# vacp2p/zerokit

Hardware: AMD Instinct MI355X
Metric: RLN Groth16 proofs/sec (BN254, h=20) (higher is better)
Workload: dtype u32 limbs (256-bit Montgomery integers, BN254 Fr/Fq; 8x32 and 9x29 forms)

## Files before the change

### zerokit_amd/csrc/prover.hip

```cpp
#include "prover.h"

#include <fcntl.h>
#include <stdlib.h>
#include <string.h>
#include <sys/stat.h>
#include <time.h>
#include <unistd.h>

#include <algorithm>
#include <atomic>
#include <chrono>
#include <deque>
#include <mutex>
#include <thread>

#include "prover_kernels.h"
#include "prover_plan.h"
#include "fq29.h"
#include "glv.h"
#include "pairing.h"
#include "poseidon.h"
#include "witness_ops.h"
#include "witness_lanes.h"
#include "witness_sched.h"
// ... 126 lines not shown
  hipStream_t sA = nullptr, sAb = nullptr, sA2 = nullptr, sB = nullptr, sB2 = nullptr, sC = nullptr;
  hipStream_t sV = nullptr;
  hipStream_t sW = nullptr;
  uint32_t seq = 0;
  hipStream_t st[ST_COUNT] = {};
  StreamPlan splan;
  float ms[PROVER_STAGES] = {0};
  DevBuf<unsigned long long> walk_clk;
  ProverTuning tune;
  DeviceCount device;
  DevBuf<GNode29> nodes29;
  DevBuf<uint32_t> consts29, slot2node;
  WitLanes witlanes;
  uint32_t nstore29 = 0, nprog29 = 0;

  uint32_t N = 0, NS = 0, NI = 0, nc = 0, ni = 0, n = 0;
  int logn = 0;
  DevBuf<uint32_t> sig2node;
  DevBuf<uint32_t> a_ptr, a_col, b_ptr, b_col;
  DevBuf<uint32_t> mv_long;
  uint32_t n_mv_long = 0;
  DevBuf<Fr> a_coef, b_coef;
  DevBuf<Fr> tw_f, tw_i, coset;
  DevBuf<G1Affine29> t1_29;
  DevBuf<G2Affine29> t2_29;
  DevBuf<uint32_t> sid1, sid2;
  struct Plan {
    DevBuf<uint32_t> rows, rsid, early_ids, late_ids, prows, prsid, pout;
    DevBuf<ChunkDesc> chunks, groups, segs, segchunks, segblocks, pchunks;
    uint32_t nchunks = 0, ngroups = 0, nseg = 0, n_early = 0, n_late = 0, npchunks = 0, nblocks = 0, maxblk = 0;
    void upload(const WalkPlan& W, hipStream_t s) {
      nchunks = (uint32_t)W.chunks.size();
      ngroups = (uint32_t)W.groups.size();
      nseg = W.nseg;
      n_early = (uint32_t)W.early_ids.size();
      n_late = (uint32_t)W.late_ids.size();
      npchunks = (uint32_t)W.pchunks.size();
      nblocks = W.nblocks;
      maxblk = W.maxblk;
      rows.assign(W.rows, s);
      rsid.assign(W.rsid, s);
      chunks.assign(W.chunks, s);
      groups.assign(W.groups, s);
      segs.assign(W.segs, s);
      segchunks.assign(W.segchunks, s);
      segblocks.assign(W.segblocks, s);
// ... 172 lines not shown
  t.verify_lanes = env_int("RLNAMD_VERIFY_LANES", 0);
  if (t.verify_lanes != 1 && t.verify_lanes != 8) t.verify_lanes = 0;
  {
    const unsigned hw = std::thread::hardware_concurrency();
    const int dflt = hw ? (int)std::min<unsigned>(t.hint_threads, std::max(1u, hw / 2)) : (int)t.hint_threads;
    t.hint_threads = (uint32_t)std::min(std::max(1, env_int("RLNAMD_HINT_THREADS", dflt)), 64);
  }
  t.hint_max_warm = (uint32_t)std::min<int>(std::max(0, env_int("RLNAMD_HINTS_WARM", (int)t.hint_max_warm)), (int)HINT_PROOFS);
  t.hint_chains = (uint32_t)std::min(std::max(0, env_int("RLNAMD_HINT_CHAINS", (int)t.hint_chains)), 1024);
  return t;
}
std::string ProverTuning::describe() const {
  char b[768];
  snprintf(b, sizeof b,
           "window_bits=%d slots=%d lanechunk=%u lanechunk_walk=%u witlanes_max=%u tiny=%u ntt_lg_max=%u partial_cache=%u lone=%d "
           "lone_small=%u hints=%u hints_warm=%u hint_threads=%u hint_chains=%u verify_lanes=%d stream_shape=%s hw_queues=%d",
           window_bits, slots, lanechunk_max, lanechunk_walk_max, witlanes_max, tiny_max, ntt_lg_max, partial_cache, lone,
           lone_small_max, hint_max, hint_max_warm, hint_threads, hint_chains, verify_lanes, stream_shape_name(stream_shape), hw_queues);
  return b;
}
const ProverTuning& Prover::tuning() const { return d_->tune; }
int Prover::device_shared() const { return (d_->device.dev >= 0 && g_provers_on_device[d_->device.dev] > 1 ? 1 : 0) | (d_->device.other_process() ? 2 : 0); }

static uint32_t bitrev(uint32_t x, int bits) {
  uint32_t r = 0;
  for (int i = 0; i < bits; i++) r |= ((x >> i) & 1u) << (bits - 1 - i);
  return r;
}

static thread_local float g_init_ms[4];
static float ms_since(std::chrono::steady_clock::time_point t0) {
  return std::chrono::duration<float, std::milli>(std::chrono::steady_clock::now() - t0).count();
}
template <class F, class Entry>
static void build_table29(const std::vector<Affine<F>>& pts, const WinSched& ws, DevBuf<Entry>& table, hipStream_t s,
                          uint32_t npaired = 0) {
  size_t npts = pts.size();
  const size_t stride = ws.stride;
  auto t_alloc = std::chrono::steady_clock::now();
  table.alloc(npts * stride);
  g_init_ms[1] += ms_since(t_alloc);
  auto t_build = std::chrono::steady_clock::now();
  DevBuf<Affine<F>> d_pts(npts);
  d_pts.upload(pts.data(), npts, s);
  size_t per_pt = stride / 2 * sizeof(F);
  size_t slab = std::max<size_t>(2, (((size_t)4 << 30) / per_pt) & ~(size_t)1);
  slab = std::min(slab, (npts + 1) & ~(size_t)1);
  DevBuf<F> scratch(slab * stride / 2);
  DevBuf<Affine<F>> tmp(slab * stride);
  for (size_t k0 = 0; k0 < npts; k0 += slab) {
    size_t cnt = std::min(slab, npts - k0);
    const size_t nrows = cnt * ws.W;
// ... 126 lines not shown
      for (size_t k = 0; k < m[r].col.size(); k++) {
        hc.push_back(graph_.signals[m[r].col[k]]);
        hv.push_back(m[r].coeff[k]);
      }
      hp[r + 1] = (uint32_t)hc.size();
    }
    ptr.assign(hp, s);
    col.assign(hc, s);
    coef.assign(hv, s);
    RLN_HIP(hipStreamSynchronize(s));
  };
  csr(zk_.a, D.a_ptr, D.a_col, D.a_coef);
  csr(zk_.b, D.b_ptr, D.b_col, D.b_coef);
  {
    std::vector<uint32_t> lr;
    for (uint32_t r = 0; r < D.nc; r++)
      if (zk_.a[r].col.size() > MV_LONG || zk_.b[r].col.size() > MV_LONG) lr.push_back(r);
    D.n_mv_long = (uint32_t)lr.size();
    D.mv_long.assign(lr, s);
    RLN_HIP(hipStreamSynchronize(s));
  }

  {
    Fr root28 = Fr::from_canonical(FR_ROOT_2_28);
    Fr g = root28;
    for (int i = 0; i < 28 - (D.logn + 1); i++) g = g.sqr();
    Fr w = g.sqr();
    Fr wi = w.inv();
    std::vector<Fr> tf(D.n / 2), ti(D.n / 2), cs(D.n);
    Fr a = Fr::one(), b = Fr::one();
    for (uint32_t k = 0; k < D.n / 2; k++) {
      tf[k] = a;
      ti[k] = b;
      a = a * w;
      b = b * wi;
    }
    Fr ninv = Fr::from_u32(D.n).inv();
    std::vector<Fr> gp(D.n);
    Fr acc = ninv;
    for (uint32_t i = 0; i < D.n; i++) {
      gp[i] = acc;
      acc = acc * g;
    }
    for (uint32_t pos = 0; pos < D.n; pos++) cs[pos] = gp[bitrev(pos, D.logn)];
    D.tw_f.assign(tf, s);
    D.tw_i.assign(ti, s);
    D.coset.assign(cs, s);
    RLN_HIP(hipStreamSynchronize(s));
  }

  {
    std::vector<uint8_t> node_known = wl_known_nodes(graph_);
    D.known.resize(D.NS);
    for (uint32_t i = 0; i < D.NS; i++) D.known[i] = node_known[graph_.signals[i]];
    {
      std::vector<uint32_t> io(96);
      for (uint32_t i = 0; i < 96; i++) io[i] = i;
      D.iota96.assign(io, s);
      RLN_HIP(hipStreamSynchronize(s));
    }
    const long want = cfg.partial_cache >= 0 ? cfg.partial_cache : (long)D.tune.partial_cache;
    D.tune.partial_cache = (uint32_t)std::max(0l, want);
    if (D.witlanes.ok && want > 0) {
      const WlCone C = wl_cone(graph_, std::move(node_known));
      std::vector<uint32_t> rows;
      for (uint32_t i = 0; i < W29.slot2node.size(); i++)
        if (C.node_known[W29.slot2node[i]]) rows.push_back(i);
      D.cone.build(C.graph, wl_cone_store_slots(C, W29.store_slot), D.nstore29, s);
      D.cone_nodes = (uint32_t)C.node_of.size();
      if (D.cone.ok && !rows.empty()) {
// ... 169 lines not shown
size_t Prover::g1_rows() const { return d_->npts1; }
size_t Prover::g2_rows() const { return d_->npts2; }

void Prover::upload(size_t n, const uint8_t* inputs, const uint8_t* rs) {
  if (n > B_) throw Error("batch larger than the prover workspace (max_batch)");
  Impl& D = *d_;
  D.sync_all();
  RLN_HIP(hipMemcpyAsync(D.inputs.p, inputs, n * D.NI * 32, hipMemcpyHostToDevice, D.sA));
  RLN_HIP(hipMemcpyAsync(D.rs.p, rs, n * 64, hipMemcpyHostToDevice, D.sA));
  RLN_HIP(hipStreamSynchronize(D.sA));
}

void Prover::upload_witness(size_t n, const uint8_t* w_le) {
  if (n > B_) throw Error("batch larger than the prover workspace (max_batch)");
  Impl& D = *d_;
  D.sync_all();
  size_t words = n * (size_t)D.NS * 8;
  if (D.wgiven.n < words) D.wgiven.alloc(words);
  RLN_HIP(hipMemcpyAsync(D.wgiven.p, w_le, words * 4, hipMemcpyHostToDevice, D.sA));
  RLN_HIP(hipStreamSynchronize(D.sA));
  D.wgiven_n = n;
}

template <bool DIF>
static void launch_ntt(Fr* data, const Fr* tw, int logn, const Fr* final_scale, uint32_t B, uint32_t nb, hipStream_t s) {
  int s0 = 0;
  while (s0 < logn) {
    const int rem = logn - s0;
    const int K = rem > 3 ? 3 : rem;
    const uint32_t groups = (1u << logn) >> K;
    dim3 block(64, 1), grid(div_up(nb, 64), groups, 3);
    const Fr* sc = (s0 + K == logn) ? final_scale : nullptr;
    switch (K) {
      case 1: hipLaunchKernelGGL((k_ntt_pass<1, DIF>), grid, block, 0, s, data, tw, logn, s0, sc, B, nb); break;
      case 2: hipLaunchKernelGGL((k_ntt_pass<2, DIF>), grid, block, 0, s, data, tw, logn, s0, sc, B, nb); break;
      default: hipLaunchKernelGGL((k_ntt_pass<3, DIF>), grid, block, 0, s, data, tw, logn, s0, sc, B, nb); break;
    }
    RLN_HIP(hipGetLastError());
    s0 += K;
  }
}

void Prover::run_async(size_t n, int mode) { enqueue(n, mode, nullptr, nullptr, nullptr); }

uint64_t Prover::submit(size_t n, const uint8_t* inputs, const uint8_t* rs, int mode, const uint8_t* partial320) {
  if (n == 0) throw Error("empty batch");
  if (!inputs || !rs) throw Error("submit: inputs and rs are required");
  if (mode == PROVE_FINISH && !partial320) throw Error("submit: finish mode needs the partial points");
  return enqueue(n, mode, inputs, rs, partial320);
}

uint64_t Prover::submit_finish(size_t n, const uint8_t* inputs, const uint8_t* rs, const uint8_t* partial320,
                               const uint64_t* handles) {
  if (n == 0) throw Error("empty batch");
  if (!inputs || !rs || !partial320) throw Error("submit_finish: inputs, rs and the partial points are required");
  return enqueue(n, PROVE_FINISH, inputs, rs, partial320, handles);
}

uint32_t Prover::hint_words() const {
  const Impl& D = *d_;
  return D.segs.ok && D.tune.hint_max > 0 ? D.n_hints * 8 : 0;
}
// ... 441 lines not shown
  } else {
    hipLaunchKernelGGL(k_witness29<false>, dim3(pg), dim3(64), WIT29_LDS_BYTES, sA, D.nodes29.p, D.nprog29,
                       D.consts29.p, (uint32_t)graph_.constants.size(), in_p, D.NI, S.V29.p, S.err.p, B, nbp, nullptr);
  }
  if (small)
    hipLaunchKernelGGL(k_v29_to_fr, dim3(div_up(D.nstore29, 64), nb), dim3(64, 1), 0, sA, S.V29.p, D.slot2node.p,
                       D.nstore29, S.V.p, B, nb, 1u);
  else
    hipLaunchKernelGGL(k_v29_to_fr, dim3(pg, D.nstore29), dim3(64, 1), 0, sA, S.V29.p, D.slot2node.p, D.nstore29, S.V.p,
                       B, nbp);
  if (hinted)
    hipLaunchKernelGGL(k_hint_check, dim3(div_up(D.n_cut, 64), nb), dim3(64), 0, sA, S.V.p, D.cut_node.p, D.cut_hint.p, D.n_cut,
                       S.h_hints, D.n_hints, B, S.err.p);
  if (D.wgiven_n) {
    if (D.wgiven_n != n || mode != PROVE_FULL) throw Error("upload_witness: the next run must be a full proof of the same batch");
    hipLaunchKernelGGL(k_scatter_witness, dim3(pg, div_up(D.NS, 4)), dim3(64, 4), 0, sA, D.wgiven.p, D.sig2node.p,
                       D.NS, S.V.p, S.err.p, B, nb);
    D.wgiven_n = 0;
  }
  RLN_HIP(hipEventRecord(S.evX, sA));
  if (early) {
    hipStream_t sR1 = sA, sR3 = lone ? D.sB : sA;
    hipLaunchKernelGGL(k_recode, dim3(div_up(D.NS + 3, 64), nb), dim3(64, 1), 0, sR1, S.V.p, D.sig2node.p, D.NS,
                       S.abc.p, D.n, rs_p, D.ws, D.ws2, S.digits.p, S.digits2.p, B, nb, 1u, 1u, dB);
    if (lone) {
      RLN_HIP(hipEventRecord(S.evW, sA));
      RLN_HIP(hipStreamWaitEvent(D.sB, S.evW, 0));
    }
    if (fused)
      hipLaunchKernelGGL(k_recode, dim3(div_up(2 * D.NS + 1, 64), nb), dim3(64, 1), 0, sR3, S.V.p, D.sig2node.p, D.NS,
                         S.abc.p, D.n, rs_p, D.ws, D.ws2, S.digits.p, S.digits2.p, B, nb, 3u, 1u, dB);
    if (!lone) {
      RLN_HIP(hipEventRecord(S.evW, sA));
      RLN_HIP(hipStreamWaitEvent(D.sB, S.evW, 0));
      RLN_HIP(hipStreamWaitEvent(D.sB2, S.evW, 0));
    }
    MARK(14, D.sB);
    walk1(D.sB, P1.early_ids.p, P1.n_early);
    RLN_HIP(hipEventRecord(S.evE, D.sB));
  }
  MARK(2, sA);
  const bool values_front = sh.values_front;
  if (values_front) {
    MARK(0, sA);
    hipLaunchKernelGGL(k_values_from_witness, dim3(pg, 5), dim3(64), 0, sA, S.V.p, D.sig2node.p, B, nbp, S.values.p);
    MARK(13, sA);
    RLN_HIP(hipEventRecord(S.evV, sA));
  }
  if (sA2 != sA) RLN_HIP(hipStreamWaitEvent(sA2, S.evX, 0));
  MARK(12, sA2);
  if (mode != PROVE_PARTIAL) {
    CsrView A{D.a_ptr.p, D.a_col.p, D.a_coef.p}, Bm{D.b_ptr.p, D.b_col.p, D.b_coef.p};
    if (small)
      hipLaunchKernelGGL(k_matvec<true>, dim3(div_up(D.n, 64) + D.n_mv_long, nb), dim3(64, 1), 0, sA2, A, Bm, S.V.p,
                         D.sig2node.p, D.nc, D.ni, D.n, S.abc.p, B, nb, D.mv_long.p, div_up(D.n, 64));
    else
      hipLaunchKernelGGL(k_matvec<false>, dim3(pg, D.n), dim3(64, 1), 0, sA2, A, Bm, S.V.p, D.sig2node.p, D.nc,
                         D.ni, D.n, S.abc.p, B, nbp);
  }
  MARK(3, sA2);
  if (mode != PROVE_PARTIAL) {
    if (sh.ntt_lds) {
      const dim3 grid(nb, D.n >> 9, 3);
      if (D.logn > 9) hipLaunchKernelGGL(k_ntt_edge<true>, grid, dim3(256), 0, sA2, S.abc.p, D.tw_i.p, D.logn, B, nb);
      hipLaunchKernelGGL(k_ntt_mid, grid, dim3(256), 0, sA2, S.abc.p, D.tw_i.p, D.tw_f.p, D.logn, D.coset.p, B, nb);
      if (D.logn > 9) hipLaunchKernelGGL(k_ntt_edge<false>, grid, dim3(256), 0, sA2, S.abc.p, D.tw_f.p, D.logn, B, nb);
      RLN_HIP(hipGetLastError());
    } else {
      launch_ntt<true>(S.abc.p, D.tw_i.p, D.logn, D.coset.p, B, nbp, sA2);
      launch_ntt<false>(S.abc.p, D.tw_f.p, D.logn, nullptr, B, nbp, sA2);
    }
    if (!early)
      hipLaunchKernelGGL(k_hquot, dim3(pg, D.n), dim3(64, 1), 0, sA2, S.abc.p, D.n, B, nbp, 0u);
  }
  MARK(4, sA2);
  hipStream_t sR = sA2;
  MARK(5, sR);
  if (early)
    hipLaunchKernelGGL(k_recode, dim3(div_up(D.n, 64), nb), dim3(64, 1), 0, sR, S.V.p, D.sig2node.p, D.NS, S.abc.p, D.n,
                       rs_p, D.ws, D.ws2, S.digits.p, S.digits2.p, B, nb, 2u, 2u, dB);
  else
    hipLaunchKernelGGL(k_recode, dim3(pg, D.NS + D.n + 3), dim3(64, 1), 0, sR, S.V.p, D.sig2node.p, D.NS,
                       S.abc.p, D.n, rs_p, D.ws, D.ws2, S.digits.p, S.digits2.p, B, nbp, 0u, 0u, dB);
  MARK(6, sR);
  if (!early) {
    RLN_HIP(hipEventRecord(S.evA, sA2));
    RLN_HIP(hipStreamWaitEvent(sB1, S.evA, 0));
    MARK(14, sB1);
  }
  hipStream_t s2 = big ? D.st[role[ROLE_WALK2]] : sh.g2_on_front ? sA : D.sB2;
  if (compact) {
    RLN_HIP(hipStreamWaitEvent(s2, S.evA, 0));
  } else if (!early) {
    RLN_HIP(hipEventRecord(S.evR, sB1));
    RLN_HIP(hipStreamWaitEvent(s2, S.evR, 0));
  }
  if (early) {
    walk1(sA2, P1.late_ids.p, P1.n_late);
    RLN_HIP(hipEventRecord(S.evR, sA2));
    RLN_HIP(hipStreamWaitEvent(D.sB, S.evR, 0));
  } else {
    walk1(sB1, nullptr, P1.nchunks);
  }
  MARK(7, sB1);
  MARK(11, s2);
  if (P2.nchunks) {
// ... 342 lines not shown
```

### zerokit_amd/csrc/prover_desc.h

```cpp
#pragma once
#include <stdint.h>

namespace rlnamd {

constexpr uint32_t OPK_RING = 0u << 30, OPK_CONST = 1u << 30, OPK_FAR = 2u << 30, OPK_MASK = 3u << 30;
constexpr uint32_t W29_STORE = 1u << 8, W29_RED = 1u << 9, W29_RARE = 1u << 10;
constexpr uint32_t W29_FMA = 25;
constexpr uint32_t WIT29_RING = 32;
constexpr uint32_t WIT29_LDS_CONSTS = 1024;
constexpr uint32_t WIT29_CH = 256;
constexpr uint32_t WIT29_LDS_BYTES = WIT29_RING * 64 * 48 + WIT29_LDS_CONSTS * 48 + 2 * WIT29_CH * 16;
constexpr double WIT29_BMAX = 7.5;
struct GNode29 {
  uint32_t w0;
  uint32_t a, b, c;
};

constexpr uint32_t MV_LONG = 8;
constexpr uint32_t SUM_TREE_LANES = 512;
struct InputSlots {
  uint32_t secret, limit, msg_id, path, path_idx, x, ext, depth;
};

struct WinSched {
  int W;
  uint32_t stride;
  uint8_t cw[32];
  uint16_t bo[32];
  uint32_t ro[32];
};

struct ChunkDesc {
  uint32_t pt_begin, pt_end;
};

constexpr uint32_t ROW_HALF2 = 1u << 31, ROW_PAIRED = 1u << 30, ROW_INDEX = ROW_PAIRED - 1;

}
```

### zerokit_amd/csrc/prover_front.hip

```cpp
#include "prover_kernels.h"

#include "glv.h"

namespace rlnamd {

__device__ __forceinline__ uint32_t wit29_addr(uint32_t enc, uint32_t lane48) {
  const uint32_t id = enc & ~OPK_MASK;
  const uint32_t cm = 0u - ((enc >> 30) & 1u);
  const uint32_t ring_a = (id % WIT29_RING) * (64 * 48), const_a = WIT29_RING * 64 * 48 + id * 48;
  return ((const_a & cm) | (ring_a & ~cm)) + (lane48 & ~cm);
}
__device__ __forceinline__ void wit29_read(Fr29& r, uint32_t addr, const uint32_t* ring) {
  const char* a = (const char*)ring + addr;
  const uint4 x = *(const uint4*)a, y = *(const uint4*)(a + 16);
  r.v[0] = x.x; r.v[1] = x.y; r.v[2] = x.z; r.v[3] = x.w;
  r.v[4] = y.x; r.v[5] = y.y; r.v[6] = y.z; r.v[7] = y.w;
  r.v[8] = *(const uint32_t*)(a + 32);
}
struct Wit29Out {
  Fr29 v;
  uint32_t e;
};
__device__ __noinline__ Wit29Out wit29_rare(uint32_t w0, uint32_t ea, uint32_t eb, uint32_t ec, const uint32_t* ring,
                                            uint32_t lane,
// ... 217 lines not shown
  }
  size_t o = (size_t)row * B + p;
  abc[o] = a;
  abc[(size_t)n * B + o] = b;
  abc[2 * (size_t)n * B + o] = (row < nc) ? a * b : Fr::zero();
}

__device__ __forceinline__ Fr29 load_fr29(const uint32_t* __restrict__ p) {
  Fr29 w;
#pragma unroll
  for (int k = 0; k < 9; k++) w.v[k] = p[k];
  return w;
}
__global__ void __launch_bounds__(256) k_consts_to29(const Fr* __restrict__ src, uint32_t* __restrict__ dst, uint32_t n) {
  uint32_t t = blockIdx.x * blockDim.x + threadIdx.x;
  if (t >= n) return;
  Fr29 v = Fr29::from_fq(src[t]);
  v.normalize();
#pragma unroll
  for (int k = 0; k < 9; k++) dst[(size_t)t * 9 + k] = v.v[k];
}
template <int K, bool DIF>
__global__ void __launch_bounds__(256, RLN_NTT_WAVES) k_ntt_pass(Fr* __restrict__ data, const Fr* __restrict__ tw, int logn, int s0,
                                                  const Fr* __restrict__ scale, uint32_t B, uint32_t nb) {
  auto tmul = [&](const Fr& a, const Fr* __restrict__ tab, uint32_t idx) -> Fr { return a * tab[idx]; };
  constexpr int R = 1 << K;
  const uint32_t n = 1u << logn;
  auto uni = [](uint32_t v) -> uint32_t { return __builtin_amdgcn_readfirstlane(v); };
  uint32_t p = blockIdx.x * 64 + threadIdx.x;
  uint32_t g = __builtin_amdgcn_readfirstlane(blockIdx.y * blockDim.y + threadIdx.y);
  if (g >= (n >> K)) return;
  if (p >= nb) return;
  Fr* x = data + (size_t)blockIdx.z * n * B + p;
  uint32_t stride, base;
  if (DIF) {
    stride = n >> (s0 + K);
    uint32_t blk = g / stride, lo = g % stride;
    base = blk * (n >> s0) + lo;
  } else {
    stride = 1u << s0;
    uint32_t blk = g / stride, lo = g % stride;
    base = blk * (stride << K) + lo;
  }
  const uint32_t lo = g % stride;
  Fr e[R];
#pragma unroll
  for (int m = 0; m < R; m++) e[m] = x[(size_t)(base + m * stride) * B];
#pragma unroll
  for (int t = 0; t < K; t++) {
    const int half = DIF ? (R >> (t + 1)) : (1 << t);
#pragma unroll
    for (int m = 0; m < R; m++) {
      if (m & half) continue;
      uint32_t j = (uint32_t)(m & (half - 1)) * stride + lo;
      uint32_t ti = DIF ? (j << (s0 + t)) : (j << (logn - 1 - (s0 + t)));
      const uint32_t tix = uni(ti);
      if (DIF) {
        Fr u = e[m], v = e[m + half];
        e[m] = u + v;
        e[m + half] = tmul(u - v, tw, tix);
      } else {
        Fr u = e[m], v = tmul(e[m + half], tw, tix);
        e[m] = u + v;
        e[m + half] = u - v;
      }
    }
  }
#pragma unroll
  for (int m = 0; m < R; m++) {
    uint32_t pos = base + m * stride;
    Fr o = e[m];
    if (scale) o = tmul(o, scale, uni(pos));
    x[(size_t)pos * B] = o;
  }
}

__global__ void __launch_bounds__(256) k_ntt_mid(Fr* __restrict__ data, const Fr* __restrict__ tw_i,
                                                 const Fr* __restrict__ tw_f, int logn, const Fr* __restrict__ scale,
                                                 uint32_t B, uint32_t nb) {
  __shared__ Fr buf[512];
  __builtin_amdgcn_s_setprio(3);
  const uint32_t p = blockIdx.x, l = threadIdx.x;
  const uint32_t n = 1u << logn, base = blockIdx.y * 512;
  if (p >= nb) return;
  Fr* x = data + (size_t)blockIdx.z * n * B + p;
  buf[l] = x[(size_t)(base + l) * B];
  buf[l + 256] = x[(size_t)(base + l + 256) * B];
  __syncthreads();
  const int E = logn - 9;
#pragma unroll 1
  for (int t = 0; t < 8; t++) {
    const uint32_t hl = 256u >> t, jl = l & (hl - 1), i0 = ((l >> (8 - t)) << (9 - t)) | jl, i1 = i0 + hl;
    const Fr u = buf[i0], v = buf[i1];
    buf[i0] = u + v;
    buf[i1] = (u - v) * tw_i[(size_t)jl << (E + t)];
    __syncthreads();
  }
// ... 43 lines not shown
  for (int t = 0; t < E; t++) {
    const int lh = DIF ? E - 1 - t : t;
    const uint32_t hm = 1u << lh, jm = q & (hm - 1), m0 = ((q >> lh) << (lh + 1)) | jm;
    const uint32_t i0 = m0 * cl + c, i1 = i0 + hm * cl;
    const size_t j = (size_t)jm * 512 + lo0 + c;
    if (DIF) {
      const Fr u = buf[i0], v = buf[i1];
      buf[i0] = u + v;
      buf[i1] = (u - v) * tw[j << t];
    } else {
      const Fr u = buf[i0], v = buf[i1] * tw[j << (logn - 1 - (9 + t))];
      buf[i0] = u + v;
      buf[i1] = u - v;
    }
    __syncthreads();
  }
#pragma unroll
  for (int k = 0; k < 2; k++) {
    const uint32_t i = l + 256 * k;
    x[(size_t)(lo0 + (i & (cl - 1)) + 512 * (i >> (9 - E))) * B] = buf[i];
  }
}

__global__ void __launch_bounds__(256) k_hquot(Fr* __restrict__ abc, uint32_t n, uint32_t B, uint32_t nb, uint32_t lg) {
  if (lg) __builtin_amdgcn_s_setprio(3);
  uint32_t p = lg ? blockIdx.y : blockIdx.x * 64 + threadIdx.x;
  uint32_t i = lg ? blockIdx.x * 64 + threadIdx.x : blockIdx.y * blockDim.y + threadIdx.y;
  if (p >= nb || i >= n) return;
  size_t o = (size_t)i * B + p;
  abc[o] = abc[o] * abc[(size_t)n * B + o] - abc[2 * (size_t)n * B + o];
}

template <int NL>
__device__ __forceinline__ void emit_digits(uint32_t* l, bool neg, const WinSched& ws, int16_t* __restrict__ out, uint32_t B) {
  uint32_t carry = 0;
#pragma unroll 1
  for (int j = 0; j < ws.W; j++) {
    const int c = ws.cw[j];
    const uint32_t mask = (c >= 32) ? 0xFFFFFFFFu : ((1u << c) - 1), E = 1u << (c - 1);
    uint32_t raw = (l[0] & mask) + carry;
#pragma unroll
    for (int i = 0; i < NL - 1; i++) l[i] = (l[i] >> c) | (l[i + 1] << (32 - c));
    l[NL - 1] >>= c;
    int d;
    if (raw > E || (raw == E && !neg)) {
      d = (int)raw - (int)(mask + 1);
      carry = 1;
    } else {
      d = (int)raw;
      carry = 0;
    }
    out[(size_t)j * B] = (int16_t)(neg ? -d : d);
  }
}
__global__ void __launch_bounds__(256) k_recode(const Fr* __restrict__ V, const uint32_t* __restrict__ sig2node,
                                                uint32_t ns, const Fr* H, uint32_t n,
                                                const uint32_t* __restrict__ rs, WinSched ws1, WinSched ws2,
                                                int16_t* __restrict__ dig1, int16_t* __restrict__ dig2, uint32_t B,
                                                uint32_t nb, uint32_t part, uint32_t lg, uint32_t dB) {
  if (lg) __builtin_amdgcn_s_setprio(3);
  uint32_t p = lg ? blockIdx.y : blockIdx.x * 64 + threadIdx.x;
  uint32_t sid = lg ? blockIdx.x * 64 + threadIdx.x : blockIdx.y * blockDim.y + threadIdx.y;
  if (part == 1) {
    if (sid >= ns + 3) return;
    if (sid >= ns) sid += n;
  } else if (part == 2) {
    if (sid >= n) return;
    sid += ns;
  } else if (part == 3) {
    if (sid >= 2 * ns + 1) return;
    sid += ns + n + 3;
  }
  if (p >= nb || sid >= 3 * ns + n + 4) return;
  Fr x;
  if (sid >= ns + n + 3) {
    const uint32_t q = sid - (ns + n + 3);
    const Fr r = Fr::from_canonical(rs + (size_t)p * 16), s = Fr::from_canonical(rs + (size_t)p * 16 + 8);
    if (q < ns)
      x = s * V[(size_t)sig2node[q] * B + p];
    else if (q < 2 * ns)
      x = r * V[(size_t)sig2node[q - ns] * B + p];
    else
      x = r * s;
  } else if (sid < ns) {
    x = V[(size_t)sig2node[sid] * B + p];
  } else if (sid < ns + n) {
    const size_t o = (size_t)(sid - ns) * B + p;
    x = lg == 2 ? H[o] * H[(size_t)n * B + o] - H[2 * (size_t)n * B + o] : H[o];
    if (lg == 2) const_cast<Fr*>(H)[o] = x;
  } else {
    Fr r = Fr::from_canonical(rs + (size_t)p * 16);
    Fr s = Fr::from_canonical(rs + (size_t)p * 16 + 8);
    uint32_t which = sid - ns - n;
    x = which == 0 ? r : which == 1 ? s : (r * s).neg();
  }
  uint32_t l[8];
  x.to_canonical(l);
  const bool g2 = sid < ns || (sid >= ns + n && sid < ns + n + 3);
  const uint32_t sid2 = sid < ns ? sid : sid - n;
  uint32_t k[2][4], neg[2];
  glv_split(l, k[0], &neg[0], k[1], &neg[1]);
#pragma unroll
  for (int h = 0; h < 2; h++) {
    uint32_t t[4];
    if (g2) {
#pragma unroll
      for (int i = 0; i < 4; i++) t[i] = k[h][i];
      emit_digits<4>(t, neg[h] != 0, ws2, dig2 + ((size_t)sid2 * 2 + h) * ws2.W * dB + p, dB);
    }
    emit_digits<4>(k[h], neg[h] != 0, ws1, dig1 + ((size_t)sid * 2 + h) * ws1.W * dB + p, dB);
  }
}


template __global__ void k_witness29<false>(const GNode29* __restrict__ nodes, uint32_t n_nodes, const uint32_t* __restrict__ consts29, uint32_t n_consts, const uint32_t* __restrict__ inputs, uint32_t n_inputs, uint4* __restrict__ V29, uint32_t* __restrict__ err, uint32_t B, uint32_t nb, unsigned long long* __restrict__ prof);
template __global__ void k_matvec<true>(CsrView A, CsrView Bm, const Fr* __restrict__ V, const uint32_t* __restrict__ sig2node, uint32_t nc, uint32_t ni, uint32_t n, Fr* __restrict__ abc, uint32_t B, uint32_t nb, const uint32_t* __restrict__ long_rows, uint32_t nshort);
template __global__ void k_matvec<false>(CsrView A, CsrView Bm, const Fr* __restrict__ V, const uint32_t* __restrict__ sig2node, uint32_t nc, uint32_t ni, uint32_t n, Fr* __restrict__ abc, uint32_t B, uint32_t nb, const uint32_t* __restrict__ long_rows, uint32_t nshort);
template __global__ void k_ntt_pass<1, true>(Fr* __restrict__ data, const Fr* __restrict__ tw, int logn, int s0, const Fr* __restrict__ scale, uint32_t B, uint32_t nb);
template __global__ void k_ntt_pass<1, false>(Fr* __restrict__ data, const Fr* __restrict__ tw, int logn, int s0, const Fr* __restrict__ scale, uint32_t B, uint32_t nb);
template __global__ void k_ntt_pass<2, true>(Fr* __restrict__ data, const Fr* __restrict__ tw, int logn, int s0, const Fr* __restrict__ scale, uint32_t B, uint32_t nb);
template __global__ void k_ntt_pass<2, false>(Fr* __restrict__ data, const Fr* __restrict__ tw, int logn, int s0, const Fr* __restrict__ scale, uint32_t B, uint32_t nb);
template __global__ void k_ntt_pass<3, true>(Fr* __restrict__ data, const Fr* __restrict__ tw, int logn, int s0, const Fr* __restrict__ scale, uint32_t B, uint32_t nb);
template __global__ void k_ntt_pass<3, false>(Fr* __restrict__ data, const Fr* __restrict__ tw, int logn, int s0, const Fr* __restrict__ scale, uint32_t B, uint32_t nb);
template __global__ void k_ntt_edge<true>(Fr* __restrict__ data, const Fr* __restrict__ tw, int logn, uint32_t B, uint32_t nb);
template __global__ void k_ntt_edge<false>(Fr* __restrict__ data, const Fr* __restrict__ tw, int logn, uint32_t B, uint32_t nb);

}
```

### zerokit_amd/csrc/prover_kernels.h

```cpp
#pragma once
#include <hip/hip_runtime.h>
#include <stdint.h>

#include <initializer_list>

#include "fq29.h"
#include "poseidon.h"
#include "prover.h"
#include "prover_desc.h"
#include "walk29.h"
#include "witness_ops.h"

namespace rlnamd {

struct CsrView {
  const uint32_t* ptr;
  const uint32_t* col;
  const Fr* coef;
};

struct TaskSel {
  uint8_t id[8];
};
inline TaskSel task_sel(std::initializer_list<uint32_t> ids) {
// ... 5 lines not shown
constexpr uint32_t SUM_TREE_LDS_G1 = SUM_TREE_LANES / 2 * 4 * 9 * 4, SUM_TREE_LDS_G2 = 2 * SUM_TREE_LDS_G1;

#ifndef RLN_NTT_WAVES
#define RLN_NTT_WAVES 1
#endif

template <bool PROF>
__global__ void __launch_bounds__(64) k_witness29(const GNode29* __restrict__ nodes, uint32_t n_nodes,
                                                  const uint32_t* __restrict__ consts29, uint32_t n_consts,
                                                  const uint32_t* __restrict__ inputs, uint32_t n_inputs,
                                                  uint4* __restrict__ V29, uint32_t* __restrict__ err, uint32_t B,
                                                  uint32_t nb, unsigned long long* __restrict__ prof);
__global__ void __launch_bounds__(64) k_v29_to_fr(const uint4* __restrict__ V29, const uint32_t* __restrict__ slot2node,
                                                  uint32_t nslots, Fr* __restrict__ V, uint32_t B, uint32_t nb,
                                                  uint32_t lg = 0);
template <bool LG>
__global__ void __launch_bounds__(256) k_matvec(CsrView A, CsrView Bm, const Fr* __restrict__ V,
                                                const uint32_t* __restrict__ sig2node, uint32_t nc, uint32_t ni,
                                                uint32_t n, Fr* __restrict__ abc, uint32_t B, uint32_t nb,
                                                const uint32_t* __restrict__ long_rows = nullptr, uint32_t nshort = 0);
__global__ void __launch_bounds__(256) k_consts_to29(const Fr* __restrict__ src, uint32_t* __restrict__ dst, uint32_t n);
template <int K, bool DIF>
__global__ void __launch_bounds__(256, RLN_NTT_WAVES) k_ntt_pass(Fr* __restrict__ data, const Fr* __restrict__ tw, int logn, int s0,
                                                  const Fr* __restrict__ scale, uint32_t B, uint32_t nb);
__global__ void __launch_bounds__(256) k_ntt_mid(Fr* __restrict__ data, const Fr* __restrict__ tw_i,
                                                 const Fr* __restrict__ tw_f, int logn, const Fr* __restrict__ scale,
                                                 uint32_t B, uint32_t nb);
template <bool DIF>
__global__ void __launch_bounds__(256) k_ntt_edge(Fr* __restrict__ data, const Fr* __restrict__ tw, int logn, uint32_t B,
                                                  uint32_t nb);
__global__ void __launch_bounds__(256) k_hquot(Fr* __restrict__ abc, uint32_t n, uint32_t B, uint32_t nb, uint32_t lg);
__global__ void __launch_bounds__(256) k_recode(const Fr* __restrict__ V, const uint32_t* __restrict__ sig2node,
                                                uint32_t ns, const Fr* H, uint32_t n,
                                                const uint32_t* __restrict__ rs, WinSched ws1, WinSched ws2,
                                                int16_t* __restrict__ dig1, int16_t* __restrict__ dig2, uint32_t B,
                                                uint32_t nb, uint32_t part, uint32_t lg, uint32_t dB);

template <class A, class E>
__global__ void __launch_bounds__(256) k_table_to29(const A* __restrict__ src, E* __restrict__ dst, size_t n, uint32_t stride,
                                                    uint32_t k0, uint32_t npaired);
template <class F>
__global__ void __launch_bounds__(64) k_sum_ranges(const XYZZ<F>* __restrict__ src, const ChunkDesc* __restrict__ ranges,
                                                   uint32_t nranges, XYZZ<F>* __restrict__ dst, uint32_t B, uint32_t nb);
template <class F, class Acc>
__global__ void __launch_bounds__(SUM_TREE_LANES) k_sum_tree(const XYZZ<F>* __restrict__ part, const ChunkDesc* __restrict__ segchunks,
                                                  XYZZ<F>* __restrict__ dst, uint32_t B, uint32_t PB, TaskSel sel);
template <class F, class Acc>
__global__ void __launch_bounds__(SUM_TREE_LANES) k_sum_blocks(const XYZZ<F>* __restrict__ part, const ChunkDesc* __restrict__ segchunks,
                                                    const ChunkDesc* __restrict__ segblocks, XYZZ<F>* __restrict__ dst, uint32_t PB,
                                                    TaskSel sel);
__global__ void __launch_bounds__(64) k_glv_fold(G1XYZZ* __restrict__ sums1, G2XYZZ* __restrict__ sums2, uint32_t nseg1,
                                                 uint32_t B, uint32_t nb, TaskSel sel);
template <class F>
__global__ void __launch_bounds__(64) k_table_build(const Affine<F>* __restrict__ pts, uint32_t npts, WinSched ws,
                                                    Affine<F>* __restrict__ table, F* __restrict__ scratch);

__global__ void __launch_bounds__(64) k_partial_out(const G1XYZZ* __restrict__ sums1, const G2XYZZ* __restrict__ sums2,
                                                    uint32_t* __restrict__ out, uint32_t B, uint32_t nb);
__global__ void __launch_bounds__(64) k_add_partial(G1XYZZ* __restrict__ sums1, G2XYZZ* __restrict__ sums2,
// ... 56 lines not shown
```

### zerokit_amd/csrc/prover_plan.cpp

```cpp
#include "prover_plan.h"

#include <stdlib.h>
#include <string.h>

#include <algorithm>

#include "glv.h"
#include "poseidon.h"
#include "witness_sched.h"

namespace rlnamd {

WinSched make_sched(int c, int wide) {
  if (c < 2 || c > 16 || wide < 0 || c + (wide > 0 ? 1 : 0) > 16) throw Error("window bits must be in [2, 16]");
  WinSched ws{};
  int W = (GlvParams::HALF_BITS - wide + c - 1) / c;
  if (wide > W) throw Error("more wide windows than windows");
  if (W > 32) throw Error("window bits too small: more than 32 windows");
  ws.W = W;
  uint32_t bit = 0, off = 0;
  for (int j = 0; j < W; j++) {
    int cw = c + (j < wide ? 1 : 0);
    ws.cw[j] = (uint8_t)cw;
    ws.bo[j] = (uint16_t)bit;
// ... 480 lines not shown
  S.small = n <= T.lanechunk_max;
  const uint32_t wl_lone_max = q.shared ? std::min(T.witlanes_max, 256u) : T.witlanes_max;
  S.wl_used = q.witlanes_ok && (S.small || (n <= wl_lone_max && S.lone));
  S.cone = mode == PROVE_FINISH && q.handles && q.inputs && S.wl_used && q.cone_ok;
  S.hinted = q.segs_ok && q.inputs && S.wl_used && !S.cone && S.lone && !q.no_hints_now &&
             n <= (q.pre_hints ? HINT_PROOFS : std::max(T.hint_max, T.hint_max_warm));
  S.probe_chains = S.hinted && !q.pre_hints && n > T.hint_max;
  S.early = S.small && mode != PROVE_PARTIAL;
  S.fused = S.lone && n <= 96 && S.early && (mode == PROVE_FULL || (mode == PROVE_FINISH && q.inputs && q.partial_points));
  S.tiny_partial = S.lone && S.small && mode == PROVE_PARTIAL && n <= T.tiny_max && n <= TINY_STRIDE && n <= T.lanechunk_walk_max;
  S.tiny = (S.fused && n <= T.tiny_max && n <= TINY_STRIDE && n <= T.lanechunk_walk_max) || S.tiny_partial;
  S.plan1 = S.tiny ? PLAN_TINY : S.fused ? PLAN_FUSED : S.small ? PLAN_SMALL : PLAN_BIG;
  S.plan2 = S.tiny ? PLAN_TINY : S.small ? PLAN_SMALL : PLAN_BIG;
  S.PB = S.tiny ? TINY_STRIDE : S.small ? q.small_stride : (uint32_t)q.capacity;
  S.walk_lp = S.early && (n > T.lanechunk_walk_max || (!S.lone && n >= 16));
  S.dB = (S.early && !S.walk_lp) ? (uint32_t)n : (uint32_t)q.capacity;
  S.g2_on_front = S.lone && S.early;
  S.values_w = (S.early || S.wl_used) && q.have_values_kernel && q.ni == 6;
  S.ntt_lds = S.small && n <= T.ntt_lg_max && q.logn >= 9 && q.logn <= 18;
  S.values_front = q.compact && !S.small && q.have_values_kernel && q.ni == 6 && (S.values_w || mode != PROVE_PARTIAL);
  return S;
}

const StreamEdge StreamPlan::edges[StreamPlan::NEDGE] = {
    {ROLE_INTERP, ROLE_VALUES}, {ROLE_INTERP, ROLE_QUOTIENT}, {ROLE_QUOTIENT, ROLE_WALK1}, {ROLE_QUOTIENT, ROLE_WALK2},
    {ROLE_WALK1, ROLE_SUMS1},   {ROLE_WALK2, ROLE_SUMS2},     {ROLE_SUMS1, ROLE_SUMS2},    {ROLE_VALUES, ROLE_SUMS2},
    {ROLE_SUMS2, ROLE_WIPE}};

int StreamPlan::busy_streams() const {
  uint32_t seen = 0;
  int n = 0;
  for (int p = 0; p < 2; p++)
    for (int r = 0; r < ROLE_COUNT; r++)
      if (r != ROLE_WIPE && !(seen >> at[p][r] & 1u)) {
        seen |= 1u << at[p][r];
        n++;
      }
  return n;
}

int hw_queues_from_env(const char* value) {
  if (!value || !*value) return 4;
  char* end = nullptr;
  const long v = strtol(value, &end, 10);
  if (end == value || *end != 0 || v < 1 || v > 1024) return 4;
  return (int)v;
// ... 46 lines not shown
```

### zerokit_amd/csrc/prover_plan.h

```cpp
#pragma once
#include <stdint.h>

#include <mutex>
#include <vector>

#include "prover.h"
#include "prover_desc.h"
#include "zkey.h"

namespace rlnamd {

constexpr uint32_t HINT_PROOFS = 64;
constexpr uint32_t TINY_STRIDE = 8;

WinSched make_sched(int c, int wide);

struct NamedInputs {
  InputSlots slots{};
  bool have_values_kernel = false;
  bool have_hint_slots = false;
  uint32_t hint_msg_off = 0, hint_msgs = 1;
};
NamedInputs find_named_inputs(const Graph& graph, uint32_t ni);

// ... 72 lines not shown
struct BatchQuery {
  size_t n = 0;
  int mode = PROVE_FULL;
  bool inputs = false, partial_points = false, handles = false, pre_hints = false;
  bool idle = true;
  bool shared = false;
  bool no_hints_now = false;
  bool witlanes_ok = false, segs_ok = false, cone_ok = false, have_values_kernel = false;
  uint32_t ni = 0;
  int logn = 0;
  size_t capacity = 0;
  uint32_t small_stride = 64;
  bool compact = false;
};
struct BatchShape {
  bool lone, small, wl_used, cone, hinted, early, fused, tiny_partial, tiny, walk_lp, g2_on_front, values_w, ntt_lds;
  bool probe_chains;
  bool values_front;
  WalkPlanKind plan1, plan2;
  uint32_t PB, dB;
};
BatchShape batch_shape(const BatchQuery& q, const ProverTuning& T);

enum StreamId : uint8_t { ST_W = 0, ST_A, ST_A2, ST_AB, ST_V, ST_B, ST_C, ST_B2, ST_COUNT };
enum StreamRole : uint8_t {
  ROLE_INTERP = 0,
  ROLE_VALUES,
  ROLE_QUOTIENT,
  ROLE_WALK1,
  ROLE_WALK2,
  ROLE_SUMS1,
  ROLE_SUMS2,
  ROLE_WIPE,
  ROLE_COUNT
};
enum StreamShape { SHAPE_AUTO = 0, SHAPE_WIDE = 1, SHAPE_COMPACT = 2 };
struct StreamEdge {
  uint8_t from, to;
};
struct StreamPlan {
  int shape = SHAPE_WIDE;
  uint8_t at[2][ROLE_COUNT] = {};
  uint8_t order[ROLE_COUNT] = {};
  bool values_front = false;
  static constexpr int NEDGE = 9;
  static const StreamEdge edges[NEDGE];
// ... 11 lines not shown
```

Before: 22010.

## Fuse NTT inverse/forward turn passes and fold quotient into recode

Restructures the fallback NTT path so the last inverse DIF pass, the coset scale, and the first forward DIT pass run in one turn kernel, cutting a full global read/write sweep and one launch. The separate k_hquot kernel is removed and the quotient computation moves into k_recode through a new hq flag. Butterflies with a unit twiddle now skip the multiply. The cost is more template variants, and the fallback path now relies on a pass list that must keep the turn width consistent.

Result: faster. 22340 (median of 6 runs) (+1.5%).

```diff
diff --git a/zerokit_amd/csrc/prover.hip b/zerokit_amd/csrc/prover.hip
--- a/zerokit_amd/csrc/prover.hip
+++ b/zerokit_amd/csrc/prover.hip
@@ -172,6 +172,7 @@
   uint32_t n_mv_long = 0;
   DevBuf<Fr> a_coef, b_coef;
   DevBuf<Fr> tw_f, tw_i, coset;
+  std::vector<NttPass> ntt_passes;
   DevBuf<G1Affine29> t1_29;
   DevBuf<G2Affine29> t2_29;
   DevBuf<uint32_t> sid1, sid2;
@@ -390,12 +391,6 @@
 const ProverTuning& Prover::tuning() const { return d_->tune; }
 int Prover::device_shared() const { return (d_->device.dev >= 0 && g_provers_on_device[d_->device.dev] > 1 ? 1 : 0) | (d_->device.other_process() ? 2 : 0); }
 
-static uint32_t bitrev(uint32_t x, int bits) {
-  uint32_t r = 0;
-  for (int i = 0; i < bits; i++) r |= ((x >> i) & 1u) << (bits - 1 - i);
-  return r;
-}
-
 static thread_local float g_init_ms[4];
 static float ms_since(std::chrono::steady_clock::time_point t0) {
   return std::chrono::duration<float, std::milli>(std::chrono::steady_clock::now() - t0).count();
@@ -568,30 +563,11 @@
   }
 
   {
-    Fr root28 = Fr::from_canonical(FR_ROOT_2_28);
-    Fr g = root28;
-    for (int i = 0; i < 28 - (D.logn + 1); i++) g = g.sqr();
-    Fr w = g.sqr();
-    Fr wi = w.inv();
-    std::vector<Fr> tf(D.n / 2), ti(D.n / 2), cs(D.n);
-    Fr a = Fr::one(), b = Fr::one();
-    for (uint32_t k = 0; k < D.n / 2; k++) {
-      tf[k] = a;
-      ti[k] = b;
-      a = a * w;
-      b = b * wi;
-    }
-    Fr ninv = Fr::from_u32(D.n).inv();
-    std::vector<Fr> gp(D.n);
-    Fr acc = ninv;
-    for (uint32_t i = 0; i < D.n; i++) {
-      gp[i] = acc;
-      acc = acc * g;
-    }
-    for (uint32_t pos = 0; pos < D.n; pos++) cs[pos] = gp[bitrev(pos, D.logn)];
-    D.tw_f.assign(tf, s);
-    D.tw_i.assign(ti, s);
-    D.coset.assign(cs, s);
+    const NttTables T = ntt_tables(D.logn);
+    D.ntt_passes = ntt_pass_list(D.logn);
+    D.tw_f.assign(T.tw_f, s);
+    D.tw_i.assign(T.tw_i, s);
+    D.coset.assign(T.coset, s);
     RLN_HIP(hipStreamSynchronize(s));
   }
 
@@ -807,22 +783,24 @@
   D.wgiven_n = n;
 }
 
-template <bool DIF>
-static void launch_ntt(Fr* data, const Fr* tw, int logn, const Fr* final_scale, uint32_t B, uint32_t nb, hipStream_t s) {
-  int s0 = 0;
-  while (s0 < logn) {
-    const int rem = logn - s0;
-    const int K = rem > 3 ? 3 : rem;
-    const uint32_t groups = (1u << logn) >> K;
-    dim3 block(64, 1), grid(div_up(nb, 64), groups, 3);
-    const Fr* sc = (s0 + K == logn) ? final_scale : nullptr;
-    switch (K) {
-      case 1: hipLaunchKernelGGL((k_ntt_pass<1, DIF>), grid, block, 0, s, data, tw, logn, s0, sc, B, nb); break;
-      case 2: hipLaunchKernelGGL((k_ntt_pass<2, DIF>), grid, block, 0, s, data, tw, logn, s0, sc, B, nb); break;
-      default: hipLaunchKernelGGL((k_ntt_pass<3, DIF>), grid, block, 0, s, data, tw, logn, s0, sc, B, nb); break;
+static void launch_ntt(const std::vector<NttPass>& passes, Fr* data, const Fr* tw_i, const Fr* tw_f, int logn, const Fr* scale,
+                       uint32_t B, uint32_t nb, hipStream_t s) {
+  for (const NttPass& ps : passes) {
+    const dim3 block(64, 1), grid(div_up(nb, 64), (1u << logn) >> ps.k, 3);
+    if (ps.kind == NTT_TURN) {
+      switch (ps.k) {
+        case 1: hipLaunchKernelGGL(k_ntt_turn<1>, grid, block, 0, s, data, tw_i, tw_f, logn, scale, B, nb); break;
+        case 2: hipLaunchKernelGGL(k_ntt_turn<2>, grid, block, 0, s, data, tw_i, tw_f, logn, scale, B, nb); break;
+        default: hipLaunchKernelGGL(k_ntt_turn<3>, grid, block, 0, s, data, tw_i, tw_f, logn, scale, B, nb); break;
+      }
+    } else if (ps.k != NTT_MAX_K) {
+      throw Error("NTT pass list: a pass that is not the turn has NTT_MAX_K levels");
+    } else if (ps.kind == NTT_DIF) {
+      hipLaunchKernelGGL((k_ntt_pass<NTT_MAX_K, true>), grid, block, 0, s, data, tw_i, logn, (int)ps.s0, B, nb);
+    } else {
+      hipLaunchKernelGGL((k_ntt_pass<NTT_MAX_K, false>), grid, block, 0, s, data, tw_f, logn, (int)ps.s0, B, nb);
     }
     RLN_HIP(hipGetLastError());
-    s0 += K;
   }
 }
 
@@ -1310,14 +1288,14 @@
   if (early) {
     hipStream_t sR1 = sA, sR3 = lone ? D.sB : sA;
     hipLaunchKernelGGL(k_recode, dim3(div_up(D.NS + 3, 64), nb), dim3(64, 1), 0, sR1, S.V.p, D.sig2node.p, D.NS,
-                       S.abc.p, D.n, rs_p, D.ws, D.ws2, S.digits.p, S.digits2.p, B, nb, 1u, 1u, dB);
+                       S.abc.p, D.n, rs_p, D.ws, D.ws2, S.digits.p, S.digits2.p, B, nb, 1u, 1u, 0u, dB);
     if (lone) {
       RLN_HIP(hipEventRecord(S.evW, sA));
       RLN_HIP(hipStreamWaitEvent(D.sB, S.evW, 0));
     }
     if (fused)
       hipLaunchKernelGGL(k_recode, dim3(div_up(2 * D.NS + 1, 64), nb), dim3(64, 1), 0, sR3, S.V.p, D.sig2node.p, D.NS,
-                         S.abc.p, D.n, rs_p, D.ws, D.ws2, S.digits.p, S.digits2.p, B, nb, 3u, 1u, dB);
+                         S.abc.p, D.n, rs_p, D.ws, D.ws2, S.digits.p, S.digits2.p, B, nb, 3u, 1u, 0u, dB);
     if (!lone) {
       RLN_HIP(hipEventRecord(S.evW, sA));
       RLN_HIP(hipStreamWaitEvent(D.sB, S.evW, 0));
@@ -1355,21 +1333,19 @@
       if (D.logn > 9) hipLaunchKernelGGL(k_ntt_edge<false>, grid, dim3(256), 0, sA2, S.abc.p, D.tw_f.p, D.logn, B, nb);
       RLN_HIP(hipGetLastError());
     } else {
-      launch_ntt<true>(S.abc.p, D.tw_i.p, D.logn, D.coset.p, B, nbp, sA2);
-      launch_ntt<false>(S.abc.p, D.tw_f.p, D.logn, nullptr, B, nbp, sA2);
-    }
-    if (!early)
-      hipLaunchKernelGGL(k_hquot, dim3(pg, D.n), dim3(64, 1), 0, sA2, S.abc.p, D.n, B, nbp, 0u);
+      launch_ntt(D.ntt_passes, S.abc.p, D.tw_i.p, D.tw_f.p, D.logn, D.coset.p, B, nbp, sA2);
+    }
   }
   MARK(4, sA2);
   hipStream_t sR = sA2;
   MARK(5, sR);
   if (early)
     hipLaunchKernelGGL(k_recode, dim3(div_up(D.n, 64), nb), dim3(64, 1), 0, sR, S.V.p, D.sig2node.p, D.NS, S.abc.p, D.n,
-                       rs_p, D.ws, D.ws2, S.digits.p, S.digits2.p, B, nb, 2u, 2u, dB);
+                       rs_p, D.ws, D.ws2, S.digits.p, S.digits2.p, B, nb, 2u, 1u, 1u, dB);
   else
     hipLaunchKernelGGL(k_recode, dim3(pg, D.NS + D.n + 3), dim3(64, 1), 0, sR, S.V.p, D.sig2node.p, D.NS,
-                       S.abc.p, D.n, rs_p, D.ws, D.ws2, S.digits.p, S.digits2.p, B, nbp, 0u, 0u, dB);
+                       S.abc.p, D.n, rs_p, D.ws, D.ws2, S.digits.p, S.digits2.p, B, nbp, 0u, 0u,
+                       mode != PROVE_PARTIAL ? 1u : 0u, dB);
   MARK(6, sR);
   if (!early) {
     RLN_HIP(hipEventRecord(S.evA, sA2));
diff --git a/zerokit_amd/csrc/prover_desc.h b/zerokit_amd/csrc/prover_desc.h
--- a/zerokit_amd/csrc/prover_desc.h
+++ b/zerokit_amd/csrc/prover_desc.h
@@ -18,6 +18,7 @@
 
 constexpr uint32_t MV_LONG = 8;
 constexpr uint32_t SUM_TREE_LANES = 512;
+constexpr int NTT_MAX_K = 3;
 struct InputSlots {
   uint32_t secret, limit, msg_id, path, path_idx, x, ext, depth;
 };
diff --git a/zerokit_amd/csrc/prover_front.hip b/zerokit_amd/csrc/prover_front.hip
--- a/zerokit_amd/csrc/prover_front.hip
+++ b/zerokit_amd/csrc/prover_front.hip
@@ -263,7 +263,7 @@
 }
 template <int K, bool DIF>
 __global__ void __launch_bounds__(256, RLN_NTT_WAVES) k_ntt_pass(Fr* __restrict__ data, const Fr* __restrict__ tw, int logn, int s0,
-                                                  const Fr* __restrict__ scale, uint32_t B, uint32_t nb) {
+                                                  uint32_t B, uint32_t nb) {
   auto tmul = [&](const Fr& a, const Fr* __restrict__ tab, uint32_t idx) -> Fr { return a * tab[idx]; };
   constexpr int R = 1 << K;
   const uint32_t n = 1u << logn;
@@ -293,27 +293,74 @@
 #pragma unroll
     for (int m = 0; m < R; m++) {
       if (m & half) continue;
+      const bool unit = (m & (half - 1)) == 0 && lo == 0;
       uint32_t j = (uint32_t)(m & (half - 1)) * stride + lo;
       uint32_t ti = DIF ? (j << (s0 + t)) : (j << (logn - 1 - (s0 + t)));
       const uint32_t tix = uni(ti);
       if (DIF) {
         Fr u = e[m], v = e[m + half];
         e[m] = u + v;
-        e[m + half] = tmul(u - v, tw, tix);
+        Fr d = u - v;
+        if (!unit) d = tmul(d, tw, tix);
+        e[m + half] = d;
       } else {
-        Fr u = e[m], v = tmul(e[m + half], tw, tix);
+        Fr u = e[m], v = e[m + half];
+        if (!unit) v = tmul(v, tw, tix);
         e[m] = u + v;
         e[m + half] = u - v;
       }
     }
   }
 #pragma unroll
-  for (int m = 0; m < R; m++) {
-    uint32_t pos = base + m * stride;
-    Fr o = e[m];
-    if (scale) o = tmul(o, scale, uni(pos));
-    x[(size_t)pos * B] = o;
-  }
+  for (int m = 0; m < R; m++) x[(size_t)(base + m * stride) * B] = e[m];
+}
+
+template <int KT>
+__global__ void __launch_bounds__(256, RLN_NTT_WAVES) k_ntt_turn(Fr* __restrict__ data, const Fr* __restrict__ tw_i,
+                                                  const Fr* __restrict__ tw_f, int logn, const Fr* __restrict__ scale,
+                                                  uint32_t B, uint32_t nb) {
+  constexpr int R = 1 << KT;
+  const uint32_t n = 1u << logn;
+  uint32_t p = blockIdx.x * 64 + threadIdx.x;
+  uint32_t g = __builtin_amdgcn_readfirstlane(blockIdx.y * blockDim.y + threadIdx.y);
+  if (g >= (n >> KT)) return;
+  if (p >= nb) return;
+  const uint32_t base = g << KT;
+  Fr* x = data + ((size_t)blockIdx.z * n + base) * B + p;
+  Fr e[R];
+#pragma unroll
+  for (int m = 0; m < R; m++) e[m] = x[(size_t)m * B];
+#pragma unroll
+  for (int t = 0; t < KT; t++) {
+    const int half = R >> (t + 1);
+#pragma unroll
+    for (int m = 0; m < R; m++) {
+      if (m & half) continue;
+      const uint32_t j = (uint32_t)(m & (half - 1));
+      Fr u = e[m], v = e[m + half];
+      e[m] = u + v;
+      Fr d = u - v;
+      if (j) d = d * tw_i[(size_t)j << (logn - KT + t)];
+      e[m + half] = d;
+    }
+  }
+#pragma unroll
+  for (int m = 0; m < R; m++) e[m] = e[m] * scale[base + m];
+#pragma unroll
+  for (int t = 0; t < KT; t++) {
+    const int half = 1 << t;
+#pragma unroll
+    for (int m = 0; m < R; m++) {
+      if (m & half) continue;
+      const uint32_t j = (uint32_t)(m & (half - 1));
+      Fr u = e[m], v = e[m + half];
+      if (j) v = v * tw_f[(size_t)j << (logn - 1 - t)];
+      e[m] = u + v;
+      e[m + half] = u - v;
+    }
+  }
+#pragma unroll
+  for (int m = 0; m < R; m++) x[(size_t)m * B] = e[m];
 }
 
 __global__ void __launch_bounds__(256) k_ntt_mid(Fr* __restrict__ data, const Fr* __restrict__ tw_i,
@@ -403,15 +450,6 @@
   }
 }
 
-__global__ void __launch_bounds__(256) k_hquot(Fr* __restrict__ abc, uint32_t n, uint32_t B, uint32_t nb, uint32_t lg) {
-  if (lg) __builtin_amdgcn_s_setprio(3);
-  uint32_t p = lg ? blockIdx.y : blockIdx.x * 64 + threadIdx.x;
-  uint32_t i = lg ? blockIdx.x * 64 + threadIdx.x : blockIdx.y * blockDim.y + threadIdx.y;
-  if (p >= nb || i >= n) return;
-  size_t o = (size_t)i * B + p;
-  abc[o] = abc[o] * abc[(size_t)n * B + o] - abc[2 * (size_t)n * B + o];
-}
-
 template <int NL>
 __device__ __forceinline__ void emit_digits(uint32_t* l, bool neg, const WinSched& ws, int16_t* __restrict__ out, uint32_t B) {
   uint32_t carry = 0;
@@ -438,7 +476,7 @@
                                                 uint32_t ns, const Fr* H, uint32_t n,
                                                 const uint32_t* __restrict__ rs, WinSched ws1, WinSched ws2,
                                                 int16_t* __restrict__ dig1, int16_t* __restrict__ dig2, uint32_t B,
-                                                uint32_t nb, uint32_t part, uint32_t lg, uint32_t dB) {
+                                                uint32_t nb, uint32_t part, uint32_t lg, uint32_t hq, uint32_t dB) {
   if (lg) __builtin_amdgcn_s_setprio(3);
   uint32_t p = lg ? blockIdx.y : blockIdx.x * 64 + threadIdx.x;
   uint32_t sid = lg ? blockIdx.x * 64 + threadIdx.x : blockIdx.y * blockDim.y + threadIdx.y;
@@ -467,8 +505,8 @@
     x = V[(size_t)sig2node[sid] * B + p];
   } else if (sid < ns + n) {
     const size_t o = (size_t)(sid - ns) * B + p;
-    x = lg == 2 ? H[o] * H[(size_t)n * B + o] - H[2 * (size_t)n * B + o] : H[o];
-    if (lg == 2) const_cast<Fr*>(H)[o] = x;
+    x = hq ? H[o] * H[(size_t)n * B + o] - H[2 * (size_t)n * B + o] : H[o];
+    if (hq) const_cast<Fr*>(H)[o] = x;
   } else {
     Fr r = Fr::from_canonical(rs + (size_t)p * 16);
     Fr s = Fr::from_canonical(rs + (size_t)p * 16 + 8);
@@ -497,12 +535,11 @@
 template __global__ void k_witness29<false>(const GNode29* __restrict__ nodes, uint32_t n_nodes, const uint32_t* __restrict__ consts29, uint32_t n_consts, const uint32_t* __restrict__ inputs, uint32_t n_inputs, uint4* __restrict__ V29, uint32_t* __restrict__ err, uint32_t B, uint32_t nb, unsigned long long* __restrict__ prof);
 template __global__ void k_matvec<true>(CsrView A, CsrView Bm, const Fr* __restrict__ V, const uint32_t* __restrict__ sig2node, uint32_t nc, uint32_t ni, uint32_t n, Fr* __restrict__ abc, uint32_t B, uint32_t nb, const uint32_t* __restrict__ long_rows, uint32_t nshort);
 template __global__ void k_matvec<false>(CsrView A, CsrView Bm, const Fr* __restrict__ V, const uint32_t* __restrict__ sig2node, uint32_t nc, uint32_t ni, uint32_t n, Fr* __restrict__ abc, uint32_t B, uint32_t nb, const uint32_t* __restrict__ long_rows, uint32_t nshort);
-template __global__ void k_ntt_pass<1, true>(Fr* __restrict__ data, const Fr* __restrict__ tw, int logn, int s0, const Fr* __restrict__ scale, uint32_t B, uint32_t nb);
-template __global__ void k_ntt_pass<1, false>(Fr* __restrict__ data, const Fr* __restrict__ tw, int logn, int s0, const Fr* __restrict__ scale, uint32_t B, uint32_t nb);
-template __global__ void k_ntt_pass<2, true>(Fr* __restrict__ data, const Fr* __restrict__ tw, int logn, int s0, const Fr* __restrict__ scale, uint32_t B, uint32_t nb);
-template __global__ void k_ntt_pass<2, false>(Fr* __restrict__ data, const Fr* __restrict__ tw, int logn, int s0, const Fr* __restrict__ scale, uint32_t B, uint32_t nb);
-template __global__ void k_ntt_pass<3, true>(Fr* __restrict__ data, const Fr* __restrict__ tw, int logn, int s0, const Fr* __restrict__ scale, uint32_t B, uint32_t nb);
-template __global__ void k_ntt_pass<3, false>(Fr* __restrict__ data, const Fr* __restrict__ tw, int logn, int s0, const Fr* __restrict__ scale, uint32_t B, uint32_t nb);
+template __global__ void k_ntt_pass<NTT_MAX_K, true>(Fr* __restrict__ data, const Fr* __restrict__ tw, int logn, int s0, uint32_t B, uint32_t nb);
+template __global__ void k_ntt_pass<NTT_MAX_K, false>(Fr* __restrict__ data, const Fr* __restrict__ tw, int logn, int s0, uint32_t B, uint32_t nb);
+template __global__ void k_ntt_turn<1>(Fr* __restrict__ data, const Fr* __restrict__ tw_i, const Fr* __restrict__ tw_f, int logn, const Fr* __restrict__ scale, uint32_t B, uint32_t nb);
+template __global__ void k_ntt_turn<2>(Fr* __restrict__ data, const Fr* __restrict__ tw_i, const Fr* __restrict__ tw_f, int logn, const Fr* __restrict__ scale, uint32_t B, uint32_t nb);
+template __global__ void k_ntt_turn<3>(Fr* __restrict__ data, const Fr* __restrict__ tw_i, const Fr* __restrict__ tw_f, int logn, const Fr* __restrict__ scale, uint32_t B, uint32_t nb);
 template __global__ void k_ntt_edge<true>(Fr* __restrict__ data, const Fr* __restrict__ tw, int logn, uint32_t B, uint32_t nb);
 template __global__ void k_ntt_edge<false>(Fr* __restrict__ data, const Fr* __restrict__ tw, int logn, uint32_t B, uint32_t nb);
 
diff --git a/zerokit_amd/csrc/prover_kernels.h b/zerokit_amd/csrc/prover_kernels.h
--- a/zerokit_amd/csrc/prover_kernels.h
+++ b/zerokit_amd/csrc/prover_kernels.h
@@ -51,19 +51,22 @@
 __global__ void __launch_bounds__(256) k_consts_to29(const Fr* __restrict__ src, uint32_t* __restrict__ dst, uint32_t n);
 template <int K, bool DIF>
 __global__ void __launch_bounds__(256, RLN_NTT_WAVES) k_ntt_pass(Fr* __restrict__ data, const Fr* __restrict__ tw, int logn, int s0,
-                                                  const Fr* __restrict__ scale, uint32_t B, uint32_t nb);
+                                                  uint32_t B, uint32_t nb);
+template <int KT>
+__global__ void __launch_bounds__(256, RLN_NTT_WAVES) k_ntt_turn(Fr* __restrict__ data, const Fr* __restrict__ tw_i,
+                                                  const Fr* __restrict__ tw_f, int logn, const Fr* __restrict__ scale,
+                                                  uint32_t B, uint32_t nb);
 __global__ void __launch_bounds__(256) k_ntt_mid(Fr* __restrict__ data, const Fr* __restrict__ tw_i,
                                                  const Fr* __restrict__ tw_f, int logn, const Fr* __restrict__ scale,
                                                  uint32_t B, uint32_t nb);
 template <bool DIF>
 __global__ void __launch_bounds__(256) k_ntt_edge(Fr* __restrict__ data, const Fr* __restrict__ tw, int logn, uint32_t B,
                                                   uint32_t nb);
-__global__ void __launch_bounds__(256) k_hquot(Fr* __restrict__ abc, uint32_t n, uint32_t B, uint32_t nb, uint32_t lg);
 __global__ void __launch_bounds__(256) k_recode(const Fr* __restrict__ V, const uint32_t* __restrict__ sig2node,
                                                 uint32_t ns, const Fr* H, uint32_t n,
                                                 const uint32_t* __restrict__ rs, WinSched ws1, WinSched ws2,
                                                 int16_t* __restrict__ dig1, int16_t* __restrict__ dig2, uint32_t B,
-                                                uint32_t nb, uint32_t part, uint32_t lg, uint32_t dB);
+                                                uint32_t nb, uint32_t part, uint32_t lg, uint32_t hq, uint32_t dB);
 
 template <class A, class E>
 __global__ void __launch_bounds__(256) k_table_to29(const A* __restrict__ src, E* __restrict__ dst, size_t n, uint32_t stride,
diff --git a/zerokit_amd/csrc/prover_plan.cpp b/zerokit_amd/csrc/prover_plan.cpp
--- a/zerokit_amd/csrc/prover_plan.cpp
+++ b/zerokit_amd/csrc/prover_plan.cpp
@@ -526,6 +526,53 @@
   return S;
 }
 
+static uint32_t bitrev(uint32_t x, int bits) {
+  uint32_t r = 0;
+  for (int i = 0; i < bits; i++) r |= ((x >> i) & 1u) << (bits - 1 - i);
+  return r;
+}
+
+NttTables ntt_tables(int logn) {
+  if (logn < 1 || logn > 27) throw Error("NTT tables: domain size out of range");
+  const uint32_t n = 1u << logn;
+  Fr g = Fr::from_canonical(FR_ROOT_2_28);
+  for (int i = 0; i < 28 - (logn + 1); i++) g = g.sqr();
+  const Fr w = g.sqr();
+  const Fr wi = w.inv();
+  NttTables T;
+  T.tw_f.resize(n / 2);
+  T.tw_i.resize(n / 2);
+  T.coset.resize(n);
+  Fr a = Fr::one(), b = Fr::one();
+  for (uint32_t k = 0; k < n / 2; k++) {
+    T.tw_f[k] = a;
+    T.tw_i[k] = b;
+    a = a * w;
+    b = b * wi;
+  }
+  if (T.tw_f[0] != Fr::one() || T.tw_i[0] != Fr::one()) throw Error("NTT tables: tw[0] is not one");
+  std::vector<Fr> gp(n);
+  Fr acc = Fr::from_u32(n).inv();
+  for (uint32_t i = 0; i < n; i++) {
+    gp[i] = acc;
+    acc = acc * g;
+  }
+  for (uint32_t pos = 0; pos < n; pos++) T.coset[pos] = gp[bitrev(pos, logn)];
+  return T;
+}
+
+int ntt_turn_width(int logn) { return logn < 1 ? 0 : (logn - 1) % NTT_MAX_K + 1; }
+
+std::vector<NttPass> ntt_pass_list(int logn) {
+  std::vector<NttPass> L;
+  if (logn < 1) return L;
+  const int kt = ntt_turn_width(logn);
+  for (int s0 = 0; s0 < logn - kt; s0 += NTT_MAX_K) L.push_back({NTT_DIF, (uint8_t)NTT_MAX_K, (uint8_t)s0});
+  L.push_back({NTT_TURN, (uint8_t)kt, (uint8_t)(logn - kt)});
+  for (int s0 = kt; s0 < logn; s0 += NTT_MAX_K) L.push_back({NTT_DIT, (uint8_t)NTT_MAX_K, (uint8_t)s0});
+  return L;
+}
+
 const StreamEdge StreamPlan::edges[StreamPlan::NEDGE] = {
     {ROLE_INTERP, ROLE_VALUES}, {ROLE_INTERP, ROLE_QUOTIENT}, {ROLE_QUOTIENT, ROLE_WALK1}, {ROLE_QUOTIENT, ROLE_WALK2},
     {ROLE_WALK1, ROLE_SUMS1},   {ROLE_WALK2, ROLE_SUMS2},     {ROLE_SUMS1, ROLE_SUMS2},    {ROLE_VALUES, ROLE_SUMS2},
diff --git a/zerokit_amd/csrc/prover_plan.h b/zerokit_amd/csrc/prover_plan.h
--- a/zerokit_amd/csrc/prover_plan.h
+++ b/zerokit_amd/csrc/prover_plan.h
@@ -118,6 +118,19 @@
 };
 BatchShape batch_shape(const BatchQuery& q, const ProverTuning& T);
 
+enum NttPassKind : uint8_t { NTT_DIF = 0, NTT_TURN, NTT_DIT };
+struct NttPass {
+  uint8_t kind;
+  uint8_t k;
+  uint8_t s0;
+};
+struct NttTables {
+  std::vector<Fr> tw_f, tw_i, coset;
+};
+NttTables ntt_tables(int logn);
+int ntt_turn_width(int logn);
+std::vector<NttPass> ntt_pass_list(int logn);
+
 enum StreamId : uint8_t { ST_W = 0, ST_A, ST_A2, ST_AB, ST_V, ST_B, ST_C, ST_B2, ST_COUNT };
 enum StreamRole : uint8_t {
   ROLE_INTERP = 0,
```
